# serhii-rieznik/metal-renderer

Hardware: AMD Instinct MI355X
Metric: Mpaths/s at 1920×1080, 4 bounces; achieved HBM GB/s vs peak; 1/2/4/8-GPU scaling (higher is better)
Workload: dtype f32

## Files before the change

metal-renderer_amd/csrc/dev_config.h:

```cpp
#pragma once

#ifndef MRT_PRECISE
#error "compile with -DMRT_PRECISE=0 or 1"
#endif
#ifndef MRT_TU
#define MRT_TU 0
#endif
#ifndef MRT_LANESTATS
#define MRT_LANESTATS 0
#endif
#define MRT_EMIT_STREAM (MRT_TU == 0 || (MRT_TU == 2 && !MRT_LANESTATS) || (MRT_TU == 1 && MRT_LANESTATS))
#define MRT_EMIT_MAIN (MRT_TU != 2)
#if MRT_PRECISE
#define MRT_NS precise
#else
#define MRT_NS fast
#endif

#ifndef MRT_BOUNCE_WAVES
#define MRT_BOUNCE_WAVES 5
#endif

#ifndef MRT_PATH_SLACK
#define MRT_PATH_SLACK 16
#endif
#ifndef MRT_LEAF_SLACK
#define MRT_LEAF_SLACK 12
#endif

#ifndef MRT_STREAM_WAVES
#define MRT_STREAM_WAVES 6
#endif
#ifndef MRT_STREAM_SPARE
#define MRT_STREAM_SPARE 1
#endif

#ifndef MRT_PATH_WAVES
#define MRT_PATH_WAVES 5
#endif
#ifndef MRT_PATH_SERVICE
#define MRT_PATH_SERVICE 32
#endif
#ifndef MRT_LDS_BLOCKS
#define MRT_LDS_BLOCKS MRT_BOUNCE_WAVES
#endif

namespace mrt { namespace MRT_NS { namespace {

constexpr int kBlock = 256;

}}}
```

metal-renderer_amd/csrc/dev_diag.h:

```cpp
#pragma once
#include <hip/hip_runtime.h>
#include <stdint.h>
#include "dev_config.h"
#include "kernels.h"

namespace mrt { namespace MRT_NS { namespace {

#if MRT_LANESTATS
constexpr int kLaneStats = 48;
__shared__ unsigned long long s_lanes[kBlock / 64][kLaneStats];
__device__ unsigned long long g_lanes[kLaneStats];
__device__ __forceinline__ void ls_add(int k, uint32_t v) {
  const uint64_t m = __ballot(1);
  if ((threadIdx.x & 63u) == (uint32_t)(__ffsll((unsigned long long)m) - 1)) s_lanes[threadIdx.x >> 6][k] += v;
}
__device__ __forceinline__ uint32_t ls_lanes() { return (uint32_t)__popcll(__ballot(1)); }
#define LS_ADD(k, v) ls_add((k), (v))
#define LS_INIT() do { if ((threadIdx.x & 63u) < (uint32_t)kLaneStats) s_lanes[threadIdx.x >> 6][threadIdx.x & 63u] = 0; } while (0)
#define LS_FLUSH() do { const uint32_t l_ = threadIdx.x & 63u; \
    if (l_ < (uint32_t)kLaneStats && s_lanes[threadIdx.x >> 6][l_]) atomicAdd(&g_lanes[l_], s_lanes[threadIdx.x >> 6][l_]); } while (0)
__device__ __forceinline__ uint64_t ls_clock() {
  uint64_t t;
  asm volatile("s_memtime %0\n\ts_waitcnt lgkmcnt(0)" : "=s"(t)::"memory");
  return t;
}
#define LS_T0() const uint64_t ls_t0_ = ls_clock()
#define LS_T1(k) do { LS_ADD((k), (uint32_t)(ls_clock() - ls_t0_)); LS_ADD((k) + 1, 1); } while (0)
#define LS_T1_LOADED(k, a, b) do { asm volatile("" ::"s"(a), "s"(b)); LS_T1(k); } while (0)
#define LS_WAIT_VM(k) do { LS_T0(); asm volatile("s_waitcnt vmcnt(0)" ::: "memory"); LS_T1(k); } while (0)
#else
#define LS_ADD(k, v) do {} while (0)
#define LS_INIT() do {} while (0)
#define LS_FLUSH() do {} while (0)
#define LS_T0() do {} while (0)
#define LS_T1(k) do {} while (0)
#define LS_T1_LOADED(k, a, b) do {} while (0)
#define LS_WAIT_VM(k) do {} while (0)
#endif

#ifndef MRT_STAMPS
#define MRT_STAMPS 0
#endif
#if MRT_STAMPS
__device__ __forceinline__ uint64_t stamp_now() {
  uint64_t t;
  __builtin_amdgcn_sched_barrier(0);
  asm volatile("s_waitcnt vmcnt(0) lgkmcnt(0)\n\ts_memtime %0\n\ts_waitcnt lgkmcnt(0)" : "=s"(t)::"memory");
  __builtin_amdgcn_sched_barrier(0);
  return t;
}
constexpr uint32_t kStampWaves = 8192;
constexpr uint32_t kStampFields = 16;
__device__ unsigned long long g_wave_t[4][kStampWaves][kStampFields];
__device__ __forceinline__ uint64_t stamp_real() {
  uint64_t t;
  asm volatile("s_memrealtime %0\n\ts_waitcnt lgkmcnt(0)" : "=s"(t)::"memory");
  return t;
}
#define STAMP_DECL() uint64_t st_acc[6] = {0, 0, 0, 0, 0, 0}; uint64_t st_prev = 0; uint64_t st_iters = 0; \
    const uint64_t st_t0 = stamp_real(); uint64_t st_why = 0, st_grab = 0, st_work = 0, st_ab = 0, \
    st_asum = 0, st_amax = 0
#define STAMP_BEGIN() do { st_prev = stamp_now(); ++st_iters; } while (0)
#define STAMP(k) do { const uint64_t t_ = stamp_now(); st_acc[k] += t_ - st_prev; st_prev = t_; } while (0)
#define STAMP_FLUSH() do { if ((threadIdx.x & 63u) == 0) { \
    const uint32_t w_ = blockIdx.x * (blockDim.x / 64u) + threadIdx.x / 64u; \
    if (w_ < kStampWaves) { unsigned long long* e_ = g_wave_t[a.bounce & 3u][w_]; \
      e_[0] = st_t0; e_[1] = stamp_real(); e_[2] = st_iters | (st_why << 32); e_[3] = st_grab; \
      e_[4] = st_work; e_[5] = st_asum; e_[6] = st_amax; e_[7] = st_grab - st_ab; \
      for (int k_ = 0; k_ < 5; ++k_) e_[8 + k_] = st_acc[k_]; e_[13] = st_entry; } } } while (0)
#define STAMP_ENTRY() const uint64_t st_entry = stamp_real()
struct StampRef { uint64_t* acc; uint64_t* prev; };
#define STAMP_REF() StampRef{st_acc, &st_prev}
#define STAMP_AT(r, k) do { const uint64_t t_ = stamp_now(); (r).acc[k] += t_ - *(r).prev; *(r).prev = t_; } while (0)
#define STAMP_ATOMIC_BEGIN() do { st_ab = stamp_real(); } while (0)
#define STAMP_EXIT(got) do { st_why = (got) == 0xFFFFFFFEu ? 2u : 1u; } while (0)
#define STAMP_GRAB() do { st_grab = stamp_real(); st_asum += st_grab - st_ab; \
    st_amax = st_grab - st_ab > st_amax ? st_grab - st_ab : st_amax; } while (0)
#define STAMP_WORK() do { st_work = stamp_real(); } while (0)
#else
#define STAMP_DECL() do {} while (0)
#define STAMP_BEGIN() do {} while (0)
#define STAMP(k) do {} while (0)
#define STAMP_FLUSH() do {} while (0)
#define STAMP_EXIT(got) do {} while (0)
#define STAMP_GRAB() do {} while (0)
#define STAMP_WORK() do {} while (0)
#define STAMP_ATOMIC_BEGIN() do {} while (0)
#define STAMP_ENTRY() do {} while (0)
struct StampRef {};
#define STAMP_REF() StampRef{}
#define STAMP_AT(r, k) do {} while (0)
#endif

#ifndef MRT_TRACE_PX
#define MRT_TRACE_PX 0
#endif
#if MRT_TRACE_PX
__device__ __forceinline__ uint32_t mdiv(uint32_t n, MagicDiv m, uint32_t d);
__device__ __forceinline__ void slot_pixel_a(uint32_t s, const BounceArgs& a, uint32_t& x, uint32_t& y);
__device__ __forceinline__ bool trace_lane(const BounceArgs& a, uint32_t tagv) {
  const uint32_t gslot = tagv & 0x7FFFFFFFu;
  const uint32_t fj = a.batch == 1u ? 0u : mdiv(gslot, a.div_slots, a.num_slots);
  uint32_t x, y;
  slot_pixel_a(gslot - fj * a.num_slots, a, x, y);
  return x == MRT_TRACE_X && y == MRT_TRACE_Y && a.frame_index + fj == MRT_TRACE_F;
}
#define MRT_TRACE(tagv, ...) do { if (trace_lane(a, (tagv))) printf(__VA_ARGS__); } while (0)
#else
#define MRT_TRACE(tagv, ...) do {} while (0)
#endif

}}}
```

metal-renderer_amd/csrc/dev_lds.h:

```cpp
#pragma once
#include "dev_math.h"
#include "kernels.h"

namespace mrt { namespace MRT_NS { namespace {

enum LdsMode { kGlobal = 0, kTopLds = 1, kAllLds = 2 };
extern __shared__ float4 g_lds[];

struct LdsCtx {
  uint32_t n_lds_nodes;
  uint32_t tri_base;
  uint32_t prim_base;
  uint32_t mat_base;
  uint32_t light_base;
  uint32_t sweep_base;
  uint32_t scratch_base;
  uint32_t stack_base;
  uint32_t* spill;
  uint32_t spill_lane;
};

__device__ __forceinline__ uint32_t* lds_u32() { return reinterpret_cast<uint32_t*>(g_lds); }

__host__ __device__ constexpr uint32_t node_stride_f4(int mode, uint32_t node_f4) {
  return (mode == kAllLds && node_f4 == 8) ? kQuadNodeF4 : node_f4;
}

__host__ __device__ inline uint32_t lds_scene_float4s(int mode, uint32_t node_f4, uint32_t nodes, uint32_t lds_nodes,
                                                      uint32_t tri_records, uint32_t prims, uint32_t mats,
                                                      uint32_t lights) {
  if (mode == kAllLds) return node_stride_f4(mode, node_f4) * nodes + 3 * tri_records + 6 * prims + 2 * mats + 7 * lights;
  if (mode == kTopLds) return node_f4 * lds_nodes;
  return 0;
}
__host__ __device__ inline uint32_t scene_nodes(const DeviceScene& sc) { return sc.num_nodes + sc.occ_nodes; }
__host__ __device__ inline uint32_t scene_tri_records(const DeviceScene& sc) { return sc.num_triangles + sc.occ_tris; }
__host__ __device__ inline uint32_t lds_scene_float4s(int mode, const DeviceScene& sc) {
  return lds_scene_float4s(mode, node_float4s(sc.width), scene_nodes(sc), sc.lds_nodes, scene_tri_records(sc),
                           sc.num_triangles, sc.num_materials, sc.num_lights + 1) +
         (mode == kAllLds ? 2 * sc.sweep_leaves : 0u);
}

__device__ __forceinline__ __amdgpu_buffer_rsrc_t buf_rsrc(const float* base) {
  return __builtin_amdgcn_make_buffer_rsrc(const_cast<float*>(base), 0, 0xFFFFFFFF, 0x00020000);
}
__device__ __forceinline__ float4 buf_ld4(__amdgpu_buffer_rsrc_t rs, uint32_t off) {
  const auto v = __builtin_amdgcn_raw_buffer_load_b128(rs, off, 0, 0);
  return make_float4(bitsf(v[0]), bitsf(v[1]), bitsf(v[2]), bitsf(v[3]));
}

template <int MODE>
__device__ __forceinline__ void fetch_node4(const DeviceScene& sc, const LdsCtx& cx, int32_t node, const RayBox& rb,
                                            float4* q) {
  if (MODE == kAllLds) {
    const uint32_t sz = fbits(rb.inv.z) >> 31;
#pragma unroll
    for (int i = 0; i < 4; ++i) q[i] = g_lds[kQuadNodeF4 * node + rb.quad_f4 + i];
    q[4] = g_lds[kQuadNodeF4 * node + rb.quad_f4 + 4 + sz];
    q[5] = g_lds[kQuadNodeF4 * node + rb.quad_f4 + 5 - sz];
    q[6] = g_lds[kQuadNodeF4 * node + rb.quad_f4 + 6];
  } else {
    const bool rowsel = MODE == kTopLds;
    const uint32_t sx = rowsel ? fbits(rb.inv.x) >> 31 : 0u, sy = rowsel ? fbits(rb.inv.y) >> 31 : 0u;
    const uint32_t sz = rowsel ? fbits(rb.inv.z) >> 31 : 0u;
    const uint32_t row[6] = {sx, 1u - sx, 2u + sy, 3u - sy, 4u + sz, 5u - sz};
    if (MODE == kAllLds || (MODE == kTopLds && (uint32_t)node < cx.n_lds_nodes)) {
#pragma unroll
      for (int i = 0; i < 6; ++i) q[i] = g_lds[8 * node + row[i]];
      q[6] = g_lds[8 * node + 6];
    } else {
      const __amdgpu_buffer_rsrc_t rs = buf_rsrc(sc.nodes);
      const uint32_t b = (uint32_t)node << 7;
#pragma unroll
      for (int i = 0; i < 6; ++i) q[i] = buf_ld4(rs, b + (row[i] << 4));
      q[6] = buf_ld4(rs, b + 96u);
    }
  }
}

template <int MODE>
__device__ __forceinline__ void fetch_tri(const DeviceScene& sc, const LdsCtx& cx, uint32_t k, float4& t0,
                                          float4& t1, float4& t2) {
  if (MODE == kAllLds) {
    t0 = g_lds[cx.tri_base + 3 * k];
    t1 = g_lds[cx.tri_base + 3 * k + 1];
    t2 = g_lds[cx.tri_base + 3 * k + 2];
  } else {
    const __amdgpu_buffer_rsrc_t rs = buf_rsrc(sc.tris);
    const uint32_t b = k * 48u;
    t0 = buf_ld4(rs, b);
    t1 = buf_ld4(rs, b + 16u);
    t2 = buf_ld4(rs, b + 32u);
  }
}

template <int MODE>
__device__ __forceinline__ float4 fetch_prim(const DeviceScene& sc, const LdsCtx& cx, uint32_t prim, uint32_t i) {
  if (MODE == kAllLds) return g_lds[cx.prim_base + 6 * prim + i];
  return reinterpret_cast<const float4*>(sc.prims)[6 * (size_t)prim + i];
}
template <int MODE>
__device__ __forceinline__ float4 fetch_mat(const DeviceScene& sc, const LdsCtx& cx, uint32_t m, uint32_t i) {
  if (MODE == kAllLds) return g_lds[cx.mat_base + 2 * m + i];
  return reinterpret_cast<const float4*>(sc.materials)[2 * m + i];
}
template <int MODE>
__device__ __forceinline__ float4 fetch_light(const DeviceScene& sc, const LdsCtx& cx, uint32_t l, uint32_t i) {
  if (MODE == kAllLds) return g_lds[cx.light_base + 7 * l + i];
  return reinterpret_cast<const float4*>(sc.lights)[7 * l + i];
}

__device__ __forceinline__ uint32_t spill_index(const LdsCtx& cx, int w) {
  return threadIdx.x * cx.spill_lane + (uint32_t)w;
}
template <int STACK>
__device__ __forceinline__ void stack_push(const LdsCtx& cx, int sp, int32_t v) {
  constexpr int kL = STACK < 0 ? -STACK : STACK;
  if (STACK > 0 || sp < kL) lds_u32()[cx.stack_base + threadIdx.x + sp * kBlock] = (uint32_t)v;
  else cx.spill[spill_index(cx, sp - kL)] = (uint32_t)v;
}
template <int STACK>
__device__ __forceinline__ int32_t stack_get(const LdsCtx& cx, int sp) {
  constexpr int kL = STACK < 0 ? -STACK : STACK;
  if (STACK > 0 || sp < kL) return (int32_t)lds_u32()[cx.stack_base + threadIdx.x + sp * kBlock];
  uint32_t v = cx.spill[spill_index(cx, sp - kL)];
  asm("" : "+v"(v));
  return (int32_t)v;
}

template <int MODE>
__device__ __forceinline__ LdsCtx stage_lds(const DeviceScene& sc, uint32_t scratch_u32, uint32_t* spill = nullptr) {
  LdsCtx cx;
  const uint32_t nf4 = node_float4s(sc.width);
  const uint32_t n_nodes = (MODE == kAllLds) ? scene_nodes(sc) : (MODE == kTopLds ? sc.lds_nodes : 0u);
  const uint32_t TR = (MODE == kAllLds) ? scene_tri_records(sc) : 0u;
  const uint32_t T = (MODE == kAllLds) ? sc.num_triangles : 0u;
  const uint32_t M = (MODE == kAllLds) ? sc.num_materials : 0u;
  const uint32_t NL = (MODE == kAllLds) ? sc.num_lights + 1 : 0u;
  const uint32_t SW = (MODE == kAllLds) ? sc.sweep_leaves : 0u;
  cx.n_lds_nodes = n_nodes;
  const uint32_t node_f4 = node_stride_f4(MODE, nf4);
  const bool copies = node_f4 != nf4;
  cx.tri_base = node_f4 * n_nodes;
  cx.prim_base = cx.tri_base + 3 * TR;
  cx.mat_base = cx.prim_base + 6 * T;
  cx.light_base = cx.mat_base + 2 * M;
  cx.sweep_base = cx.light_base + 7 * NL;
  const uint32_t f4 = cx.sweep_base + 2 * SW;
  cx.scratch_base = 4 * f4;
  cx.stack_base = cx.scratch_base + ((scratch_u32 + 3) & ~3u);
  cx.spill_lane = sc.max_stack;
  cx.spill = spill ? spill + (size_t)blockIdx.x * kBlock * cx.spill_lane : nullptr;
  if (MODE != kGlobal) {
    const float4* src[6] = {reinterpret_cast<const float4*>(sc.nodes), reinterpret_cast<const float4*>(sc.tris),
                            reinterpret_cast<const float4*>(sc.prims), reinterpret_cast<const float4*>(sc.materials),
                            reinterpret_cast<const float4*>(sc.lights), reinterpret_cast<const float4*>(sc.sweep)};
    const uint32_t base[6] = {0u, cx.tri_base, cx.prim_base, cx.mat_base, cx.light_base, cx.sweep_base};
    const uint32_t len[6] = {nf4 * n_nodes, 3 * TR, 6 * T, 2 * M, 7 * NL, 2 * SW};
    for (int r = copies ? 1 : 0; r < 6; ++r)
      for (uint32_t i = threadIdx.x; i < len[r]; i += kBlock) g_lds[base[r] + i] = src[r][i];
    if (copies) {
      for (uint32_t i = threadIdx.x; i < node_f4 * n_nodes; i += kBlock) {
        const uint32_t node = i / node_f4, rem = i % node_f4;
        const uint32_t quad = rem / kQuadCopyF4, row = rem % kQuadCopyF4;
        const uint32_t axis = row >> 1;
        const uint32_t flip = axis < 2 ? (quad >> axis) & 1u : 0u;
        const uint32_t src_row = row < 6 ? 2 * axis + ((row & 1u) ^ flip) : 6u;
        g_lds[i] = src[0][8 * node + src_row];
      }
    }
    __syncthreads();
  }
  return cx;
}

}}}
```

metal-renderer_amd/csrc/dev_shadow.h:

```cpp
#pragma once
#include "dev_traverse.h"

namespace mrt { namespace MRT_NS { namespace {

__device__ __forceinline__ int32_t shadow_root(const DeviceScene& sc, V3 o, bool graze) {
  const int32_t main_root = __builtin_amdgcn_readfirstlane(sc.root);
  if (sc.occ_planes == 0) return main_root;
  const int32_t occ_root = __builtin_amdgcn_readfirstlane(sc.occ_root);
  bool inside = !graze;
  for (uint32_t k = 0; k < sc.occ_planes; ++k) {
    const float* p = sc.occ_plane[k];
    inside &= fmaf(p[0], o.x, fmaf(p[1], o.y, fmaf(p[2], o.z, -p[3]))) <= -sc.occ_margin;
  }
  return inside ? occ_root : main_root;
}
__device__ __forceinline__ int32_t shadow_root_select(const DeviceScene& sc, V3 o, bool graze) {
  if (sc.occ_planes == 0 || graze) return sc.root;
  bool inside = true;
  for (uint32_t k = 0; k < sc.occ_planes; ++k) {
    const float* p = sc.occ_plane[k];
    inside &= fmaf(p[0], o.x, fmaf(p[1], o.y, fmaf(p[2], o.z, -p[3]))) <= -sc.occ_margin;
  }
  return inside ? sc.occ_root : sc.root;
}

template <int MODE>
__device__ __forceinline__ bool lights_occlude(const DeviceScene& sc, const LdsCtx& cx, V3 o, V3 d, uint32_t target,
                                               uint32_t tl, float tT) {
  bool occ = false;
  for (uint32_t j = 0; j + 1 < sc.num_lights; ++j) {
    const uint32_t k = j < tl ? j : j + 1u;
    const float4 LB = fetch_light<MODE>(sc, cx, k, 1), LD = fetch_light<MODE>(sc, cx, k, 3);
    const float4 LF = fetch_light<MODE>(sc, cx, k, 5);
    const uint32_t prim = fbits(LD.w);
    const V3 p0 = mk(LB);
    float t, u, v;
    const bool ok = tri_bary(o, d, p0, sub(mk(LD), p0), sub(mk(LF), p0), t, u, v);
    occ |= ok & (prim != target) & (t >= 0.0f) & (t <= tT) & ((t < tT) | (prim < target));
  }
  return occ;
}

template <int MODE>
__device__ __forceinline__ bool face_occludes(const DeviceScene& sc, const LdsCtx& cx, V3 o, V3 d, uint32_t pair,
                                              uint32_t target, float tT) {
  bool occ = false;
#pragma unroll
  for (int j = 0; j < 2; ++j) {
    const uint32_t prim = (pair >> (16 * j)) & 0xFFFFu;
    if (prim != 0xFFFFu) {
      const V3 p0 = mk(fetch_prim<MODE>(sc, cx, prim, 0)), p1 = mk(fetch_prim<MODE>(sc, cx, prim, 1));
      const V3 p2 = mk(fetch_prim<MODE>(sc, cx, prim, 2));
      float t, u, v;
      const bool ok = tri_bary(o, d, p0, sub(p1, p0), sub(p2, p0), t, u, v);
      occ |= ok & (prim != target) & (t >= 0.0f) & (t <= tT) & ((t < tT) | (prim < target));
    }
  }
  return occ;
}

template <int MODE>
__device__ __forceinline__ bool convex_occlusion(const DeviceScene& sc, const LdsCtx& cx, V3 o, V3 d, uint32_t target,
                                                 float tT, uint32_t origin) {
  const uint32_t own = fbits(fetch_prim<MODE>(sc, cx, origin, 2).w);
  const V3 own_n = mk(fetch_prim<MODE>(sc, cx, origin, 3).w, fetch_prim<MODE>(sc, cx, origin, 4).w,
                      fetch_prim<MODE>(sc, cx, origin, 5).w);
  const uint32_t own_skip = ((own != 0u) & (dot(d, own_n) >= kConvexLeaveDot)) ? (own - 1u) >> 3 : 0xFFFFFFFFu;
  bool occluded = false;
  for (uint32_t c = 0; c < sc.conv_count; ++c) {
    const float* B = sc.conv_obb[c];
    float t0 = 0.0f, t1 = tT;
    uint32_t fin = 8u, fout = 8u;
#pragma unroll
    for (uint32_t a = 0; a < 3; ++a) {
      const float nd = (B[3 * a] * d.x + B[3 * a + 1] * d.y) + B[3 * a + 2] * d.z;
      const float no = (B[3 * a] * o.x + B[3 * a + 1] * o.y) + B[3 * a + 2] * o.z;
      const float inv = m_rcp(nd);
      const float tlo = (B[9 + 2 * a] - no) * inv, thi = (B[10 + 2 * a] - no) * inv;
      const bool pos = (fbits(nd) >> 31) == 0u;
      const float tn = pos ? tlo : thi, tf = pos ? thi : tlo;
      const bool in_ = tn > t0, out_ = tf < t1;
      t0 = in_ ? tn : t0;
      fin = in_ ? (pos ? 2u * a : 2u * a + 1u) : fin;
      t1 = out_ ? tf : t1;
      fout = out_ ? (pos ? 2u * a + 1u : 2u * a) : fout;
    }
    const bool leaves_own = own_skip == c;
    if ((t0 <= t1) & !leaves_own & !occluded) {
      uint32_t pin = 0xFFFFFFFFu, pout = 0xFFFFFFFFu;
#pragma unroll
      for (uint32_t k = 0; k < 6; ++k) {
        pin = fin == k ? sc.conv_face_tris[c][k] : pin;
        pout = fout == k ? sc.conv_face_tris[c][k] : pout;
      }
      bool hit = face_occludes<MODE>(sc, cx, o, d, pin != 0xFFFFFFFFu ? pin : pout, target, tT);
      if (!hit & (pin != 0xFFFFFFFFu)) hit = face_occludes<MODE>(sc, cx, o, d, pout, target, tT);
      if (!hit) {
#pragma unroll
        for (uint32_t k = 0; k < 6; ++k)
          if (!hit & (k != fin) & (k != fout)) hit = face_occludes<MODE>(sc, cx, o, d, sc.conv_face_tris[c][k], target, tT);
      }
      occluded |= hit;
    }
  }
  return occluded;
}

template <int STACK, int MODE>
__device__ __forceinline__ bool trace_occluded(const DeviceScene& sc, const LdsCtx& cx, V3 o, V3 d, uint32_t target,
                                               uint32_t tl, float t_target, bool graze, uint32_t origin,
                                               uint32_t dbg = 0u) {
  Hit h;
  h.t = t_target;
  h.found = false;
  LS_T0();
  int32_t root = shadow_root(sc, o, graze);
#if MRT_LANESTATS
  asm volatile("" ::"v"(root));
  LS_T1(40);
#endif
  const bool via_occ = root == sc.occ_root;
  if (sc.conv_count && via_occ) {
    if (!(dbg & 512u) && convex_occlusion<MODE>(sc, cx, o, d, target, t_target, origin)) return true;
    root = kDone;
  }
  if (sc.occ_lights && via_occ && !(dbg & 1024u) && lights_occlude<MODE>(sc, cx, o, d, target, tl, t_target)) return true;
  return traverse<STACK, MODE, true>(sc, cx, o, d, 0.0f, h, target, root);
}

template <int MODE>
__device__ __forceinline__ bool origin_occludes(const DeviceScene& sc, const LdsCtx& cx, V3 o, V3 d, uint32_t prim,
                                                uint32_t target, float tT) {
  if (!sc.origin_test) return false;
  const V3 p0 = mk(fetch_prim<MODE>(sc, cx, prim, 0)), p1 = mk(fetch_prim<MODE>(sc, cx, prim, 1));
  const V3 p2 = mk(fetch_prim<MODE>(sc, cx, prim, 2));
  float t, u, v;
  const bool ok = tri_bary(o, d, p0, sub(p1, p0), sub(p2, p0), t, u, v);
  return ok & (prim != target) & (t >= 0.0f) & (t <= tT) & ((t < tT) | (prim < target));
}

template <int STACK, int MODE>
__device__ bool shadow_reaches_target(const DeviceScene& sc, const LdsCtx& cx, V3 o, V3 d, uint32_t target,
                                      uint32_t origin, bool graze, uint32_t dbg = 0u) {
  const float4 P1 = fetch_prim<MODE>(sc, cx, target, 1);
  const V3 p0 = mk(fetch_prim<MODE>(sc, cx, target, 0)), p1 = mk(P1);
  const V3 p2 = mk(fetch_prim<MODE>(sc, cx, target, 2));
  float tT, u, v;
  if (!tri_test(o, d, p0, sub(p1, p0), sub(p2, p0), 0.0f, __builtin_inff(), tT, u, v)) return false;
  if (!(tT >= kDistanceEpsilon)) return false;
  if (!(dbg & 128u) && origin_occludes<MODE>(sc, cx, o, d, origin, target, tT)) return false;
  if (dbg & 32u) return true;
  return !trace_occluded<STACK, MODE>(sc, cx, o, d, target, fbits(P1.w), tT, graze, origin, dbg);
}

template <int MODE>
__device__ __forceinline__ bool last_bounce_light_hit(const DeviceScene& sc, const LdsCtx& cx, V3 o, V3 d, Hit& h,
                                                      bool& graze) {
  h.t = __builtin_inff();
  h.u = h.v = 0.0f;
  h.prim = 0xFFFFFFFFu;
  h.found = false;
  float gd = 0.0f, gn = 1.0f;
  for (uint32_t k = 0; k < sc.num_lights; ++k) {
    const float4 LB = fetch_light<MODE>(sc, cx, k, 1), LD = fetch_light<MODE>(sc, cx, k, 3);
    const float4 LF = fetch_light<MODE>(sc, cx, k, 5);
    const uint32_t prim = fbits(LD.w);
    const V3 p0 = mk(LB), e1 = sub(mk(LD), p0), e2 = sub(mk(LF), p0);
    float t, u, v;
    const bool ok = tri_bary(o, d, p0, e1, e2, t, u, v);
    const bool hit = ok & (t >= 0.0f) & (t <= h.t);
    if (hit & (!h.found | (t < h.t) | (prim < h.prim))) {
      h.found = true;
      h.t = t;
      h.u = u;
      h.v = v;
      h.prim = prim;
      const V3 n = tcross(e1, e2);
      const float dn = tdot(d, n);
      gd = dn * dn;
      gn = tdot(n, n);
    }
  }
  if (h.found && h.t < kDistanceEpsilon) h.found = false;
  graze = !(gd >= sc.occ_cos_min2 * gn);
  return h.found;
}

}}}
```

metal-renderer_amd/csrc/kern_bounce.h:

```cpp
#pragma once
#include "dev_diag.h"
#include "dev_shade.h"
#include "dev_shadow.h"
#include "dev_sweep.h"

namespace mrt { namespace MRT_NS { namespace {

__device__ __forceinline__ uint32_t block_exclusive_scan(uint32_t* v, uint32_t n, uint32_t* wave_tmp) {
  const uint32_t tid = threadIdx.x, lane = tid & 63u, wave = tid >> 6;
  const uint32_t per = (n + kBlock - 1) / kBlock;
  const uint32_t b = tid * per, e = min(n, b + per);
  uint32_t local = 0;
  for (uint32_t i = b; i < e; ++i) local += v[i];
  uint32_t incl = local;
  for (int off = 1; off < 64; off <<= 1) {
    const uint32_t up = __shfl_up(incl, off);
    if ((int)lane >= off) incl += up;
  }
  if (lane == 63) wave_tmp[wave] = incl;
  __syncthreads();
  uint32_t wave_prefix = 0, total = 0;
  for (uint32_t w = 0; w < kBlock / 64; ++w) {
    if (w < wave) wave_prefix += wave_tmp[w];
    total += wave_tmp[w];
  }
  uint32_t run = wave_prefix + incl - local;
  for (uint32_t i = b; i < e; ++i) {
    const uint32_t x = v[i];
    v[i] = run;
    run += x;
  }
  __syncthreads();
  return total;
}

__device__ __forceinline__ void wait_vmem() {
  asm volatile("" ::: "memory");
  __builtin_amdgcn_s_waitcnt(0x0F70);
  asm volatile("" ::: "memory");
}

template <int STACK, int MODE, bool WAVEQ = false, bool CAM = false, bool LIST = false>
__device__ __forceinline__ uint32_t bounce_wave(const DeviceScene& sc, const LdsCtx& cx, const BounceArgs& a,
                                               uint32_t bounce, bool active, uint32_t idx, uint32_t slot,
                                               const RayQueue& in_q, const RayQueue& out_q, uint32_t* cursor,
                                               uint32_t out_base, uint32_t cap,
                                               StampRef st, uint32_t& recycled) {
  const uint32_t lane = threadIdx.x & 63u;
  const bool last = (bounce + 1 == a.max_path_length);
  LS_ADD(14, 1);
  LS_ADD(15, (uint32_t)__popcll(__ballot(active)));
  PathState s;
  uint32_t tag = 0;
  uint32_t resume = 0, unfinished = 0;
  recycled = 0;
  uint32_t pblk = 0xFFFFFFFFu;
  if (active) {
    if (bounce == 0) {
      const uint32_t fj = a.batch == 1u ? 0u : __builtin_amdgcn_readfirstlane(mdiv(idx, a.div_slots, a.num_slots));
      uint32_t x, y;
      slot_pixel_l<LIST, true>(idx - fj * a.num_slots, a, x, y);
      active = (x < a.width) && (y < a.height);
      if (active) {
        tag = idx;
        pblk = (x / kPrimaryBlock) + (y / kPrimaryBlock) * a.primary_bx;
        const float4 ns = noise_table(a, fj, 0u)[(x % kNoiseDim) + (y % kNoiseDim) * kNoiseDim];
        camera_ray<CAM>(x, y, a.width, a.height, ns, noise_table(a, fj, 0u), a.camera, s.o, s.d);
      }
    } else {
      const float4 q0 = in_q.plane[0][slot], q1 = in_q.plane[1][slot];
      if (WAVEQ) LS_WAIT_VM(34);
      s.o = mk(q0);
      tag = fbits(q0.w);
      s.d = mk(q1);
      s.prevDiffuse = (tag >> 31) ? 1.0f : 0.0f;
      if (WAVEQ) resume = fbits(q1.w);
    }
  }
  STAMP_AT(st, 0);
  Hit h;
  h.found = false;
  bool listed = false;
  if (bounce == 0 && a.primary) {
    const uint32_t b0 = __builtin_amdgcn_readfirstlane(pblk);
    const bool uniform = b0 != 0xFFFFFFFFu && __ballot(active && pblk != b0) == 0;
    LS_T0();
    const PrimaryWords words = (PrimaryWords)(uintptr_t)a.primary;
    const uint32_t hd = uniform ? words[b0] : kPrimaryFallback;
#if MRT_LANESTATS
    asm volatile("" ::"s"(hd));
    if (WAVEQ && uniform) LS_T1(38);
#endif
    const uint32_t cnt = hd & 0xFFu;
    if (cnt != kPrimaryFallback) {
      listed = true;
      LS_ADD(18, 1);
      LS_ADD(19, (uint32_t)__popcll(__ballot(active)));
      if (active) primary_nearest<MODE>(sc, cx, words + (hd >> 8), cnt, s.o, s.d, h);
    }
  }
  if (active && !listed) {
    if (last && sc.light_shortcut && !(a.flags & kShadeDebugMaterial)) {
      bool graze;
      if (last_bounce_light_hit<MODE>(sc, cx, s.o, s.d, h, graze)) {
        Hit hh;
        hh.t = h.t;
        hh.found = false;
        const int32_t root = shadow_root(sc, s.o, graze);
        if (!(a.debug & 64u) && traverse<STACK, MODE, true>(sc, cx, s.o, s.d, 0.0f, hh, h.prim, root)) h.found = false;
      }
    } else if (WAVEQ && MODE == kAllLds && sc.sweep_leaves) {
      h.t = __builtin_inff();
      h.u = h.v = 0.0f;
      h.prim = 0xFFFFFFFFu;
      if (resume) {
        const float4 ph = a.out_q.plane[0][slot];
        h.t = ph.x;
        h.u = ph.y;
        h.v = ph.z;
        h.prim = fbits(ph.w);
        h.found = h.prim != 0xFFFFFFFFu;
      }
      const uint32_t pops = __builtin_amdgcn_readfirstlane(bounce == 0 ? 0xFFFFFFFFu : sc.sweep_cap);
      unfinished = sweep_nearest<MODE, true>(sc, cx, s.o, s.d, 0.0f, h, pops, resume);
    } else {
      h = trace_nearest<STACK, MODE>(sc, cx, s.o, s.d, 0.0f, __builtin_inff());
    }
  }
  STAMP_AT(st, 1);
  const uint32_t gslot = tag & 0x7FFFFFFFu;
  if (active) {
    if (bounce == 0) {
      s.T = mk(1.0f, 1.0f, 1.0f);
      s.R = mk(0.0f, 0.0f, 0.0f);
      s.pdf = 1.0f;
      s.prevDiffuse = 0.0f;
      s.ior = 1.00029f;
    } else {
      const float4 q2 = in_q.plane[2][slot], q3 = in_q.plane[3][slot];
      if (WAVEQ) LS_WAIT_VM(36);
      s.T = mk(q2);
      s.pdf = q2.w;
      s.R = mk(q3);
      s.ior = q3.w;
    }
  }
  if (WAVEQ) {
    const uint64_t rmask = __ballot(unfinished != 0u);
    if (rmask) {
      LS_ADD(32, (uint32_t)__popcll(rmask));
      asm volatile("s_waitcnt vmcnt(0)" ::: "memory");
      if (unfinished) {
        const uint32_t r = slot - lane + lanes_below_in(rmask);
        in_q.plane[0][r] = make_float4(s.o.x, s.o.y, s.o.z, bitsf(tag));
        in_q.plane[1][r] = make_float4(s.d.x, s.d.y, s.d.z, bitsf(unfinished));
        in_q.plane[2][r] = make_float4(s.T.x, s.T.y, s.T.z, s.pdf);
        in_q.plane[3][r] = make_float4(s.R.x, s.R.y, s.R.z, s.ior);
        a.out_q.plane[0][r] = make_float4(h.t, h.u, h.v, bitsf(h.prim));
      }
      recycled = (uint32_t)__popcll(rmask);
      active = active && !unfinished;
    }
    if (__ballot(resume != 0u)) LS_ADD(33, 1);
  }
  const bool hit_ok = active && h.found && !(h.t < kDistanceEpsilon);
  ShadowRay sh;
  sh.valid = false;
  if (__ballot(hit_ok)) {
    LS_ADD(12, 1);
    LS_ADD(13, (uint32_t)__popcll(__ballot(hit_ok)));
  }
  if (hit_ok) {
    const uint32_t fj = a.batch == 1u ? 0u : mdiv(gslot, a.div_slots, a.num_slots);
    uint32_t x, y;
    slot_pixel_l<LIST>(gslot - fj * a.num_slots, a, x, y);
    const uint32_t back = (bounce % 3u) == 0 ? 0u : ((bounce % 3u) == 1 ? 2u : 1u);
    const float4 ns = noise_table(a, fj, back)[shade_noise_cell(x, y, bounce, a.frame_index + fj)];
    if (a.debug & 2u) {
      s.o = add(s.o, mul(s.d, h.t * 0.999f));
      s.d = mk(-s.d.x, -s.d.y, -s.d.z);
    } else {
      shade_hit<MODE>(sc, cx, h, s, ns, bounce, a.max_path_length, !last, sh, (a.flags & kShadeDebugMaterial) != 0);
    }
  }
  STAMP_AT(st, 2);
  if (WAVEQ) wait_vmem();
  if (active && (!hit_ok || last)) a.radiance[gslot] = make_float4(s.R.x, s.R.y, s.R.z, 0.0f);
  const bool alive = hit_ok && !last;
  const bool cls1 = !WAVEQ && (s.prevDiffuse == 0.0f) && !(a.debug & 16u);
  const uint64_t mask0 = __ballot(alive && !cls1), mask1 = __ballot(alive && cls1);
  uint32_t o = 0, wrote = 0;
  if (mask0 | mask1) {
    uint32_t w0 = 0, w1 = 0;
    if (!WAVEQ && lane == 0) {
      if (mask0) w0 = atomicAdd(&cursor[0], (uint32_t)__popcll(mask0));
      if (mask1) w1 = atomicAdd(&cursor[1], (uint32_t)__popcll(mask1));
    }
    w0 = __shfl(w0, 0);
    w1 = __shfl(w1, 0);
    o = cls1 ? out_base + cap - 1u - (w1 + lanes_below_in(mask1)) : out_base + w0 + lanes_below_in(mask0);
    if (alive && !(a.debug & 4u)) {
      out_q.plane[0][o] = make_float4(s.o.x, s.o.y, s.o.z, bitsf(gslot | (s.prevDiffuse != 0.0f ? 0x80000000u : 0u)));
      out_q.plane[1][o] = make_float4(s.d.x, s.d.y, s.d.z, 0.0f);
      out_q.plane[2][o] = make_float4(s.T.x, s.T.y, s.T.z, s.pdf);
    }
    wrote = (uint32_t)__popcll(mask0 | mask1);
  }
  STAMP_AT(st, 3);
  if (__ballot(sh.valid)) {
    LS_ADD(16, (uint32_t)__popcll(__ballot(sh.valid)));
    LS_ADD(17, 1);
  }
  if (sh.valid && ((a.debug & 1u) || shadow_reaches_target<STACK, MODE>(sc, cx, sh.o, sh.d, sh.target, h.prim, sh.graze, a.debug))) {
    s.R = add(s.R, sh.L);
  }
  if (alive && !(a.debug & 4u)) out_q.plane[3][o] = make_float4(s.R.x, s.R.y, s.R.z, s.ior);
  STAMP_AT(st, 4);
  return wrote;
}

template <int STACK, int MODE, bool CAM = false>
__global__ __launch_bounds__(kBlock, MRT_BOUNCE_WAVES) void bounce_kernel(DeviceScene sc, BounceArgs a) {
  __shared__ uint32_t s_wave[kBlock / 64];
  __shared__ uint32_t s_cursor[2], s_res, s_closed;
  STAMP_ENTRY();
  span_begin(a);
  LS_INIT();
  const uint32_t tid = threadIdx.x;
  const uint32_t G = gridDim.x;
  const uint32_t nseg = (a.bounce == 0) ? 0u : a.in_segments;
  const LdsCtx cx = stage_lds<MODE>(sc, nseg + 1, a.stack_spill);
  uint32_t* seg = lds_u32() + cx.scratch_base;
  if (tid == 0) s_cursor[0] = s_cursor[1] = s_res = s_closed = 0;

  uint32_t N, in_chunk = 0;
  if (a.bounce == 0) {
    N = a.num_slots * a.batch;
    __syncthreads();
  } else {
    for (uint32_t i = tid; i < nseg; i += kBlock) seg[i] = a.in_seg_count[i];
    __syncthreads();
    N = block_exclusive_scan(seg, nseg, s_wave);
    if (tid == 0) seg[nseg] = N;
    __syncthreads();
    in_chunk = *a.in_chunk;
  }
  const uint32_t chunk = ((N + G - 1) / G + kBlock - 1) / kBlock * kBlock;
  const bool dynamic = (a.debug & 8u) == 0;
  const uint32_t cap = dynamic ? chunk + kSegSlack : chunk;
  const uint32_t out_base = blockIdx.x * cap;
  const uint32_t rlen = ((N + kGrabRanges - 1) / kGrabRanges + kGrab - 1) / kGrab * kGrab;
  uint32_t cur_range = blockIdx.x % kGrabRanges, ranges_left = kGrabRanges;
  uint32_t static_base = blockIdx.x * kBlock + (tid & ~63u);

  const uint32_t lane = tid & 63u;

  STAMP_DECL();
  for (;;) {
    uint32_t start, end, niter;
    if (dynamic) {
      uint32_t got = 0xFFFFFFFFu;
      STAMP_ATOMIC_BEGIN();
      if (lane == 0) {
        if (atomicAdd(&s_res, kGrab) + kGrab <= cap) {
          while (ranges_left) {
            const uint32_t r0 = cur_range * rlen;
            if (r0 < N && !(__hip_atomic_load(&s_closed, __ATOMIC_RELAXED, __HIP_MEMORY_SCOPE_WORKGROUP) & (1u << cur_range))) {
              const uint32_t i = atomicAdd(a.grab + cur_range * kGrabStride, kGrab);
              if (i < rlen && r0 + i < N) { got = r0 + i; break; }
              atomicOr(&s_closed, 1u << cur_range);
            }
            cur_range = cur_range + 1 == kGrabRanges ? 0u : cur_range + 1;
            --ranges_left;
          }
          if (got == 0xFFFFFFFFu) atomicSub(&s_res, kGrab);
        } else {
          got = 0xFFFFFFFEu;
        }
      }
      got = __builtin_amdgcn_readfirstlane(got);
      if (got >= 0xFFFFFFFEu) { STAMP_EXIT(got); break; }
      cur_range = __builtin_amdgcn_readfirstlane(cur_range);
      ranges_left = __builtin_amdgcn_readfirstlane(ranges_left);
      STAMP_GRAB();
      start = got;
      end = min(N, cur_range * rlen + rlen);
      niter = kGrab / 64;
    } else {
      if (static_base >= N) break;
      start = static_base;
      end = N;
      niter = 1;
      static_base += G * kBlock;
    }
    uint32_t wrote = 0;
    for (uint32_t it = 0; it < niter; ++it) {
      const uint32_t idx = start + it * 64u + lane;
      bool active = idx < end;
      uint32_t slot = 0;
      if (active && a.bounce != 0) {
        uint32_t lo = 0, hi = nseg;
        while (hi - lo > 1) { const uint32_t mid = (lo + hi) >> 1; if (seg[mid] <= idx) lo = mid; else hi = mid; }
        const uint32_t g_in = nseg >> 1;
        slot = lo < g_in ? lo * in_chunk + (idx - seg[lo])
                         : (lo - g_in) * in_chunk + in_chunk - (seg[lo + 1] - seg[lo]) + (idx - seg[lo]);
      }
      STAMP_BEGIN();
      uint32_t none;
      wrote += bounce_wave<STACK, MODE, false, CAM>(sc, cx, a, a.bounce, active, idx, slot, a.in_q, a.out_q, s_cursor,
                                               out_base, cap, STAMP_REF(), none);
    }
    STAMP_WORK();
    if (dynamic && lane == 0) atomicSub(&s_res, kGrab - wrote);
  }
  STAMP_FLUSH();
  __syncthreads();
  if (tid == 0) {
    a.out_seg_count[blockIdx.x] = s_cursor[0];
    a.out_seg_count[G + blockIdx.x] = s_cursor[1];
    const uint32_t total = s_cursor[0] + s_cursor[1];
    if (total) atomicAdd(a.out_total, total);
    if (blockIdx.x == 0) *a.out_chunk = cap;
  }
  LS_FLUSH();
  span_end(a);
}

}}}
```

Baseline: 16040.

## Plan convex-solid shadow tests with slab entry face first and LDS face table

Restructures convex occluder shadow testing. A first pass computes the OBB slab intersections for every solid and packs a compact plan recording the first crossed solid, its entry and exit faces, and which other solids are crossed. The entry face of the first solid is tested first, and the remaining faces and solids are checked only when a lane in the wavefront still needs them, with the face-to-triangle table staged in LDS. The aim is to cut the number of face tests and the divergent global loads per shadow ray, at the cost of extra LDS space (which may affect occupancy) and a second pass over the slabs. Lane-stat counters split by bounce are also added for diagnostics.

Result: faster. 16340 (median of 6 runs) (+1.8%).

```diff
diff --git a/metal-renderer_amd/csrc/dev_config.h b/metal-renderer_amd/csrc/dev_config.h
--- a/metal-renderer_amd/csrc/dev_config.h
+++ b/metal-renderer_amd/csrc/dev_config.h
@@ -45,6 +45,10 @@
 #define MRT_LDS_BLOCKS MRT_BOUNCE_WAVES
 #endif
 
+#ifndef MRT_CONVEX_LOOP
+#define MRT_CONVEX_LOOP 0
+#endif
+
 namespace mrt { namespace MRT_NS { namespace {
 
 constexpr int kBlock = 256;
diff --git a/metal-renderer_amd/csrc/dev_diag.h b/metal-renderer_amd/csrc/dev_diag.h
--- a/metal-renderer_amd/csrc/dev_diag.h
+++ b/metal-renderer_amd/csrc/dev_diag.h
@@ -7,8 +7,9 @@
 namespace mrt { namespace MRT_NS { namespace {
 
 #if MRT_LANESTATS
-constexpr int kLaneStats = 48;
+constexpr int kLaneStats = 52;
 __shared__ unsigned long long s_lanes[kBlock / 64][kLaneStats];
+__shared__ uint32_t s_lane_split[kBlock / 64];
 __device__ unsigned long long g_lanes[kLaneStats];
 __device__ __forceinline__ void ls_add(int k, uint32_t v) {
   const uint64_t m = __ballot(1);
@@ -16,7 +17,14 @@
 }
 __device__ __forceinline__ uint32_t ls_lanes() { return (uint32_t)__popcll(__ballot(1)); }
 #define LS_ADD(k, v) ls_add((k), (v))
-#define LS_INIT() do { if ((threadIdx.x & 63u) < (uint32_t)kLaneStats) s_lanes[threadIdx.x >> 6][threadIdx.x & 63u] = 0; } while (0)
+__device__ __forceinline__ void ls_split(uint32_t cls) {
+  const uint64_t m = __ballot(1);
+  if ((threadIdx.x & 63u) == (uint32_t)(__ffsll((unsigned long long)m) - 1)) s_lane_split[threadIdx.x >> 6] = cls;
+}
+#define LS_SPLIT(cls) ls_split((cls))
+#define LS_ADD_SPLIT(k, v) ls_add((k) + 2 * (int)s_lane_split[threadIdx.x >> 6], (v))
+#define LS_INIT() do { if ((threadIdx.x & 63u) < (uint32_t)kLaneStats) s_lanes[threadIdx.x >> 6][threadIdx.x & 63u] = 0; \
+    if ((threadIdx.x & 63u) == 0u) s_lane_split[threadIdx.x >> 6] = 0; } while (0)
 #define LS_FLUSH() do { const uint32_t l_ = threadIdx.x & 63u; \
     if (l_ < (uint32_t)kLaneStats && s_lanes[threadIdx.x >> 6][l_]) atomicAdd(&g_lanes[l_], s_lanes[threadIdx.x >> 6][l_]); } while (0)
 __device__ __forceinline__ uint64_t ls_clock() {
@@ -30,6 +38,8 @@
 #define LS_WAIT_VM(k) do { LS_T0(); asm volatile("s_waitcnt vmcnt(0)" ::: "memory"); LS_T1(k); } while (0)
 #else
 #define LS_ADD(k, v) do {} while (0)
+#define LS_SPLIT(cls) do {} while (0)
+#define LS_ADD_SPLIT(k, v) do {} while (0)
 #define LS_INIT() do {} while (0)
 #define LS_FLUSH() do {} while (0)
 #define LS_T0() do {} while (0)
diff --git a/metal-renderer_amd/csrc/dev_lds.h b/metal-renderer_amd/csrc/dev_lds.h
--- a/metal-renderer_amd/csrc/dev_lds.h
+++ b/metal-renderer_amd/csrc/dev_lds.h
@@ -14,6 +14,7 @@
   uint32_t mat_base;
   uint32_t light_base;
   uint32_t sweep_base;
+  uint32_t conv_base;
   uint32_t scratch_base;
   uint32_t stack_base;
   uint32_t* spill;
@@ -33,12 +34,13 @@
   if (mode == kTopLds) return node_f4 * lds_nodes;
   return 0;
 }
+__host__ __device__ inline uint32_t conv_table_float4s(const DeviceScene& sc) { return 2u * sc.conv_count; }
 __host__ __device__ inline uint32_t scene_nodes(const DeviceScene& sc) { return sc.num_nodes + sc.occ_nodes; }
 __host__ __device__ inline uint32_t scene_tri_records(const DeviceScene& sc) { return sc.num_triangles + sc.occ_tris; }
 __host__ __device__ inline uint32_t lds_scene_float4s(int mode, const DeviceScene& sc) {
   return lds_scene_float4s(mode, node_float4s(sc.width), scene_nodes(sc), sc.lds_nodes, scene_tri_records(sc),
                            sc.num_triangles, sc.num_materials, sc.num_lights + 1) +
-         (mode == kAllLds ? 2 * sc.sweep_leaves : 0u);
+         (mode == kAllLds ? 2 * sc.sweep_leaves + conv_table_float4s(sc) : 0u);
 }
 
 __device__ __forceinline__ __amdgpu_buffer_rsrc_t buf_rsrc(const float* base) {
@@ -146,7 +148,9 @@
   cx.mat_base = cx.prim_base + 6 * T;
   cx.light_base = cx.mat_base + 2 * M;
   cx.sweep_base = cx.light_base + 7 * NL;
-  const uint32_t f4 = cx.sweep_base + 2 * SW;
+  const uint32_t CV = (MODE == kAllLds) ? conv_table_float4s(sc) : 0u;
+  cx.conv_base = 4 * (cx.sweep_base + 2 * SW);
+  const uint32_t f4 = cx.sweep_base + 2 * SW + CV;
   cx.scratch_base = 4 * f4;
   cx.stack_base = cx.scratch_base + ((scratch_u32 + 3) & ~3u);
   cx.spill_lane = sc.max_stack;
@@ -159,6 +163,8 @@
     const uint32_t len[6] = {nf4 * n_nodes, 3 * TR, 6 * T, 2 * M, 7 * NL, 2 * SW};
     for (int r = copies ? 1 : 0; r < 6; ++r)
       for (uint32_t i = threadIdx.x; i < len[r]; i += kBlock) g_lds[base[r] + i] = src[r][i];
+    for (uint32_t i = threadIdx.x; i < 4 * CV; i += kBlock)
+      lds_u32()[cx.conv_base + i] = (i & 7u) < 6u ? sc.conv_face_tris[i >> 3][i & 7u] : 0xFFFFFFFFu;
     if (copies) {
       for (uint32_t i = threadIdx.x; i < node_f4 * n_nodes; i += kBlock) {
         const uint32_t node = i / node_f4, rem = i % node_f4;
diff --git a/metal-renderer_amd/csrc/dev_shadow.h b/metal-renderer_amd/csrc/dev_shadow.h
--- a/metal-renderer_amd/csrc/dev_shadow.h
+++ b/metal-renderer_amd/csrc/dev_shadow.h
@@ -1,5 +1,6 @@
 #pragma once
 #include "dev_traverse.h"
+#include "shadow_plan.h"
 
 namespace mrt { namespace MRT_NS { namespace {
 
@@ -60,8 +61,8 @@
 }
 
 template <int MODE>
-__device__ __forceinline__ bool convex_occlusion(const DeviceScene& sc, const LdsCtx& cx, V3 o, V3 d, uint32_t target,
-                                                 float tT, uint32_t origin) {
+__device__ __forceinline__ bool convex_occlusion_loop(const DeviceScene& sc, const LdsCtx& cx, V3 o, V3 d,
+                                                      uint32_t target, float tT, uint32_t origin) {
   const uint32_t own = fbits(fetch_prim<MODE>(sc, cx, origin, 2).w);
   const V3 own_n = mk(fetch_prim<MODE>(sc, cx, origin, 3).w, fetch_prim<MODE>(sc, cx, origin, 4).w,
                       fetch_prim<MODE>(sc, cx, origin, 5).w);
@@ -87,6 +88,7 @@
     }
     const bool leaves_own = own_skip == c;
     if ((t0 <= t1) & !leaves_own & !occluded) {
+      LS_ADD_SPLIT(48, 1);
       uint32_t pin = 0xFFFFFFFFu, pout = 0xFFFFFFFFu;
 #pragma unroll
       for (uint32_t k = 0; k < 6; ++k) {
@@ -101,6 +103,69 @@
           if (!hit & (k != fin) & (k != fout)) hit = face_occludes<MODE>(sc, cx, o, d, sc.conv_face_tris[c][k], target, tT);
       }
       occluded |= hit;
+    }
+  }
+  return occluded;
+}
+
+__device__ __forceinline__ bool convex_slabs(const DeviceScene& sc, uint32_t c, V3 o, V3 d, float tT, uint32_t& fin,
+                                             uint32_t& fout) {
+  const float* B = sc.conv_obb[c];
+  float t0 = 0.0f, t1 = tT;
+  fin = 8u;
+  fout = 8u;
+#pragma unroll
+  for (uint32_t a = 0; a < 3; ++a) {
+    const float nd = (B[3 * a] * d.x + B[3 * a + 1] * d.y) + B[3 * a + 2] * d.z;
+    const float no = (B[3 * a] * o.x + B[3 * a + 1] * o.y) + B[3 * a + 2] * o.z;
+    const float inv = m_rcp(nd);
+    const float tlo = (B[9 + 2 * a] - no) * inv, thi = (B[10 + 2 * a] - no) * inv;
+    const bool pos = (fbits(nd) >> 31) == 0u;
+    const float tn = pos ? tlo : thi, tf = pos ? thi : tlo;
+    const bool in_ = tn > t0, out_ = tf < t1;
+    t0 = in_ ? tn : t0;
+    fin = in_ ? (pos ? 2u * a : 2u * a + 1u) : fin;
+    t1 = out_ ? tf : t1;
+    fout = out_ ? (pos ? 2u * a + 1u : 2u * a) : fout;
+  }
+  return t0 <= t1;
+}
+
+template <int MODE>
+__device__ __forceinline__ bool convex_occlusion(const DeviceScene& sc, const LdsCtx& cx, V3 o, V3 d, uint32_t target,
+                                                 float tT, uint32_t origin) {
+  const uint32_t own = fbits(fetch_prim<MODE>(sc, cx, origin, 2).w);
+  const V3 own_n = mk(fetch_prim<MODE>(sc, cx, origin, 3).w, fetch_prim<MODE>(sc, cx, origin, 4).w,
+                      fetch_prim<MODE>(sc, cx, origin, 5).w);
+  const uint32_t own_skip = ((own != 0u) & (dot(d, own_n) >= kConvexLeaveDot)) ? (own - 1u) >> 3 : 0xFFFFFFFFu;
+  uint32_t plan = 0u;
+  for (uint32_t c = 0; c < sc.conv_count; ++c) {
+    uint32_t fin, fout;
+    const bool crosses = convex_slabs(sc, c, o, d, tT, fin, fout);
+    plan = shadow_plan_add(plan, c, crosses & (own_skip != c), fin, fout);
+  }
+  bool occluded = false;
+  if (shadow_plan_has(plan)) {
+    LS_ADD_SPLIT(48, 1);
+    const uint32_t at = shadow_plan_pair_index(shadow_plan_solid(plan), shadow_plan_first_face(plan));
+    occluded = face_occludes<MODE>(sc, cx, o, d, lds_u32()[cx.conv_base + at], target, tT);
+  }
+  const bool more = shadow_plan_has(plan) & !occluded;
+  if (__ballot(more)) {
+    const uint32_t crossed = more ? shadow_plan_crossed(plan) : 0u;
+    for (uint32_t c = 0; c < sc.conv_count; ++c) {
+      if (((crossed >> c) & 1u) & !occluded) {
+        uint32_t fin, fout;
+        convex_slabs(sc, c, o, d, tT, fin, fout);
+        uint32_t todo = shadow_plan_todo(plan, c);
+        bool hit = false;
+        while ((todo != 0u) & !hit) {
+          const uint32_t k = shadow_plan_next_face(fin, fout, todo);
+          todo &= ~(1u << k);
+          hit = face_occludes<MODE>(sc, cx, o, d, lds_u32()[cx.conv_base + shadow_plan_pair_index(c, k)], target, tT);
+        }
+        occluded |= hit;
+      }
     }
   }
   return occluded;
@@ -121,7 +186,10 @@
 #endif
   const bool via_occ = root == sc.occ_root;
   if (sc.conv_count && via_occ) {
-    if (!(dbg & 512u) && convex_occlusion<MODE>(sc, cx, o, d, target, t_target, origin)) return true;
+    LS_ADD_SPLIT(49, 1);
+    if (!(dbg & 512u) && (MODE == kAllLds && !MRT_CONVEX_LOOP ? convex_occlusion<MODE>(sc, cx, o, d, target, t_target, origin)
+                                          : convex_occlusion_loop<MODE>(sc, cx, o, d, target, t_target, origin)))
+      return true;
     root = kDone;
   }
   if (sc.occ_lights && via_occ && !(dbg & 1024u) && lights_occlude<MODE>(sc, cx, o, d, target, tl, t_target)) return true;
diff --git a/metal-renderer_amd/csrc/kern_bounce.h b/metal-renderer_amd/csrc/kern_bounce.h
--- a/metal-renderer_amd/csrc/kern_bounce.h
+++ b/metal-renderer_amd/csrc/kern_bounce.h
@@ -210,6 +210,7 @@
   if (__ballot(sh.valid)) {
     LS_ADD(16, (uint32_t)__popcll(__ballot(sh.valid)));
     LS_ADD(17, 1);
+    LS_SPLIT(bounce == 0u ? 0u : 1u);
   }
   if (sh.valid && ((a.debug & 1u) || shadow_reaches_target<STACK, MODE>(sc, cx, sh.o, sh.d, sh.target, h.prim, sh.graze, a.debug))) {
     s.R = add(s.R, sh.L);
diff --git a/metal-renderer_amd/csrc/shadow_plan.h b/metal-renderer_amd/csrc/shadow_plan.h
--- /dev/null
+++ b/metal-renderer_amd/csrc/shadow_plan.h
@@ -0,0 +1,54 @@
+#pragma once
+#include <cstdint>
+
+#if defined(__HIPCC__)
+#define MRT_PLAN_FN __host__ __device__ __forceinline__
+#else
+#define MRT_PLAN_FN inline
+#endif
+
+namespace mrt {
+
+constexpr uint32_t kPlanNoFace = 8u;
+constexpr uint32_t kPlanHas = 1u << 10;
+constexpr uint32_t kPlanLaterShift = 12u;
+constexpr uint32_t kPlanAllFaces = 0x3Fu;
+constexpr uint32_t kPlanRow = 8u;
+
+MRT_PLAN_FN uint32_t shadow_plan_add(uint32_t plan, uint32_t c, bool crossed, uint32_t fin, uint32_t fout) {
+  const uint32_t first = fin | (fout << 4) | (c << 8) | kPlanHas;
+  const uint32_t later = plan | ((1u << kPlanLaterShift) << c);
+  return crossed ? ((plan & kPlanHas) ? later : first) : plan;
+}
+
+MRT_PLAN_FN bool shadow_plan_has(uint32_t plan) { return (plan & kPlanHas) != 0u; }
+MRT_PLAN_FN uint32_t shadow_plan_fin(uint32_t plan) { return plan & 15u; }
+MRT_PLAN_FN uint32_t shadow_plan_fout(uint32_t plan) { return (plan >> 4) & 15u; }
+MRT_PLAN_FN uint32_t shadow_plan_solid(uint32_t plan) { return (plan >> 8) & 3u; }
+MRT_PLAN_FN uint32_t shadow_plan_later(uint32_t plan) { return (plan >> kPlanLaterShift) & 15u; }
+
+MRT_PLAN_FN uint32_t shadow_plan_first_face(uint32_t plan) {
+  const uint32_t fin = shadow_plan_fin(plan);
+  return fin != kPlanNoFace ? fin : shadow_plan_fout(plan);
+}
+
+MRT_PLAN_FN uint32_t shadow_plan_pair_index(uint32_t solid, uint32_t face) {
+  return solid * kPlanRow + (face < kPlanRow - 1u ? face : kPlanRow - 1u);
+}
+
+MRT_PLAN_FN uint32_t shadow_plan_crossed(uint32_t plan) {
+  return shadow_plan_has(plan) ? (shadow_plan_later(plan) | (1u << shadow_plan_solid(plan))) : 0u;
+}
+
+MRT_PLAN_FN uint32_t shadow_plan_todo(uint32_t plan, uint32_t c) {
+  const uint32_t tested = shadow_plan_solid(plan) == c ? (1u << shadow_plan_first_face(plan)) : 0u;
+  return kPlanAllFaces & ~tested;
+}
+
+MRT_PLAN_FN uint32_t shadow_plan_next_face(uint32_t fin, uint32_t fout, uint32_t todo) {
+  if ((todo >> fin) & 1u) return fin;
+  if ((todo >> fout) & 1u) return fout;
+  return (uint32_t)__builtin_ctz(todo);
+}
+
+}
```
